# CMU-SAFARI/AirLift

Measured on AMD Instinct MI355X. Metric: reads/sec remapped (150 bp PE), higher is better.
Workload: dtype u8/int32 (int8 SW lanes, u64 hashes)

## Files before the change

airlift_amd/csrc/al_kernels_chain.hip:

```cpp
#include <hip/hip_runtime.h>
#include <stdint.h>
#include "al_internal.h"
#include "al_device.h"

#define CT_TILE 1024
#define CT_SEGS (CT_TILE / 2)
#define CT_FRAGS 32
#define CT_NU_CAP 64
#define CT_CLIN_N 512
#define CT_NONE 0xffffu

#define R_XLO(r) ((uint32_t)(r) & 0xffffu)
#define R_Q(r) ((int32_t)((uint32_t)(r) >> 16 & 0xfffu))
#define R_SEG(r) ((int32_t)((uint32_t)(r) >> 28 & 1u))
#define R_F(r) ((int32_t)(int16_t)((r) >> 32))
#define R_P(r) ((uint32_t)((r) >> 48))
#define ROW_B30 (1u << 30)
#define ROW_B31 (1u << 31)

struct CtFrag {
	uint64_t aoff;
	uint32_t f, na;
	int32_t mdx, mdy; uint32_t drlim;
	uint32_t start;
// ... 684 lines not shown
	const uint32_t f = fb_list[v]; const uint32_t n_u = v_nu[v];
	const uint64_t *su = v_u + v_a_off[v] + v; uint64_t *du = u_all + a_off[f] + f; uint32_t *duo = uo_all + a_off[f] + f;
	uint32_t run = 0;
	for (uint32_t c0 = 0; c0 < n_u; c0 += 64) {
		const uint32_t c = c0 + lane; const uint64_t uc = c < n_u ? su[c] : 0ULL; const uint32_t cnt = (uint32_t)uc;
		uint32_t incl = cnt; for (int d = 1; d < 64; d <<= 1) { const uint32_t t = __shfl_up(incl, d); if (lane >= d) incl += t; }
		if (c < n_u) { du[c] = uc; duo[c] = run + incl - cnt; }
		run += __shfl(incl, 63);
	}
	const AlAnchor *sc = v_chained + v_a_off[v]; AlAnchor *dc = chained + a_off[f];
	for (uint32_t t = lane; t < run; t += 64) dc[t] = sc[t];
	if (lane == 0) frag_nu[f] = n_u;
}

__global__ void __launch_bounds__(256)
k_frag_meta(const uint32_t *__restrict__ frag_first, const uint32_t *__restrict__ rd_len, int n_frag, uint32_t *__restrict__ meta)
{
	const int f = blockIdx.x * blockDim.x + threadIdx.x;
	if (f >= n_frag) return;
	const uint32_t r0 = frag_first[f], r1 = frag_first[f + 1];
	uint32_t q = 0; for (uint32_t r = r0; r < r1; ++r) q += rd_len[r];
	meta[f] = q | (r1 - r0 > 1 ? 1u << 31 : 0u);
}
```

airlift_amd/csrc/al_runtime.h:

```cpp
#pragma once
#include <hip/hip_runtime.h>
#include <stdio.h>
#include <vector>
#include <string>
#include <thread>
#include <chrono>
#include "al_internal.h"
#include "al_stream_plan.h"
#include "al_env.h"
#include "al_devmem.h"

template <typename T> struct DevBuf {
	T *p = nullptr; size_t cap = 0;
	int ensure(size_t n, bool keep = false, hipStream_t s = 0, int line = __builtin_LINE(), const char *file = __builtin_FILE())
	{
		if (n <= cap) return 0;
		al_alloc_site() = AlAllocSite{file, line};
		const size_t big_div = (size_t)al_env().grow_div;
		const size_t ncap = n + (n * sizeof(T) >= ((size_t)256 << 20) ? n / big_div : n / 4) + 64;
		T *np = nullptr;
		if (!keep && p) { al_dev_free(p); p = nullptr; cap = 0; }
		if (al_dev_malloc((void **)&np, ncap * sizeof(T)) != hipSuccess) {
			(void)hipGetLastError();
			fprintf(stderr, "[airlift] device allocation of %zu bytes failed\n", ncap * sizeof(T)); al_nomem_flag() = true; return -1;
// ... 61 lines not shown
	std::vector<uint32_t> h_rd_len, h_frag_first, h_frag_hash;
	std::vector<uint64_t> h_rd_off, h_mini_off;
	std::vector<uint32_t> h_rd_seq;
	std::vector<uint8_t> h_flip;

	DevBuf<uint32_t> rd_seq, rd_len, frag_first, frag_hash, mini_cnt, frag_nm, frag_na, frag_nu, rechain_list, rechain_sorted, tmp_u32;
	DevBuf<uint64_t> rd_off, mini_off, a_off, u, ws_u64, tmp_u64, tmp_u64b;
	DevBuf<uint32_t> uo;
	DevBuf<uint64_t> big_k0, big_k1;
	DevBuf<AlAnchor> v_anchors, v_chained; DevBuf<uint64_t> v_u, v_a_off, v_first64; DevBuf<uint32_t> v_na, v_nseg, v_first, v_rd_len, v_order, v_nu, fbk_list;
	DevBuf<uint64_t> d_uslot; DevBuf<uint32_t> d_rel, d_fragid, cmp_list, ctie, frag_meta, chain_cls;
	DevBuf<int32_t> frag_rep, ws_i32;
	DevBuf<AlAnchor> mini, heap_ws, anchors, chained;
	DevBuf<AlMatch> match;
	DevBuf<unsigned long long> counters;
	DevBuf<uint8_t> scan_tmp;
	DevBuf<uint8_t> big_tmp;
	DevBuf<uint32_t> chain_key, chain_idx, chain_idx2, tie_list, lb_buf;
	DevBuf<AlAnchor> chain_tmp; DevBuf<uint64_t> u_tmp, okey_tmp, seg_first, seg_first0, vs_off, big_off, big_toff;
	DevBuf<uint64_t> vs_res;
	DevBuf<uint32_t> seg_cnt, seg_cnt0, seg_t1, vs_na, vs_meta, vs_cls, seg_key, seg_idx, seg_ord, fb_list, fb2_list, fb3_list, big_na, big_nt, big_tent, big_cuts, tie_frags, tie_sorted, heap_cnt;
	AlChainScratch tie2;
	uint64_t n_chain_fallback = 0;
	uint64_t chain_who[AL_CHAIN_WHO_N] = {};
	DevBuf<unsigned long long> seed_cnt;
	uint64_t seed_who[AL_SEED_WHO_N] = {};
	bool seed_tap_pass1 = false;
	int max_qlen_sum = 0;
	int max_rd_len = 0;
	bool attr_chain_order = false, attr_regs_heavy = false;
	bool no_taps = false;
	bool dev_batch = false;
	DevBuf<uint64_t> a_off_p1; DevBuf<uint32_t> frag_na_p1; DevBuf<int32_t> frag_rep_p1;
	uint64_t n_anchor_total = 0, n_anchor_pass1 = 0;
	double anchor_grow_hw = 1.3;
	uint32_t n_rechain = 0;

	DevBuf<AlReg> regs0, regs;
	DevBuf<uint32_t> reg_cnt, cigar;
	DevBuf<uint64_t> reg_off, cig_off;
	DevBuf<uint8_t> align_ws;
	DevBuf<AlAnchor> seg_a;
	DevBuf<uint64_t> seg_u;
	uint64_t n_regs_cap_total = 0, n_cigar_cap_total = 0;
	bool ran = false;
	uint64_t stat_bytes_in = 0;
	uint32_t stat_n_slow = 0;
	unsigned long long stat_dp_jobs[10] = {}, stat_dp_tbases[10] = {};
	al_batch_stat_t stat;
};

int al_upload_index(const al_idx_t *mi, int device, AlDevIndex *out);
int al_windows_prepare(al_ctx_t *c, int n_tok, int read_len);
// ... 69 lines not shown
```

airlift_amd/csrc/al_runtime.hip:

```cpp
#include <hip/hip_runtime.h>
#include <stdio.h>
#include <stdlib.h>
#include <string.h>
#include <cstring>
#include <algorithm>
#include <functional>
#include <thread>
#include <chrono>
#include "al_internal.h"
#include "al_device.h"
#include <mutex>
#include <vector>
#include "al_runtime.h"
#include "al_prim.h"
#include "al_dev_sort.h"
#include "al_io.h"

extern "C" __global__ void k_sketch(const uint32_t *, const uint64_t *, const uint32_t *, const uint64_t *, AlAnchor *, uint32_t *, int, int, int, int);
extern "C" __global__ void k_seed(const uint64_t *, int, const uint32_t *, const uint32_t *, const uint64_t *, AlAnchor *, const uint32_t *, AlMatch *, uint32_t *, uint32_t *, int32_t *, const uint32_t *, int, int, int, uint32_t *);
#ifndef AL_SPEC_CAP
#define AL_SPEC_CAP 512
#endif
struct SpecOut { AlMatch *match; uint32_t *meta; uint32_t *cnt; uint64_t *cand; uint32_t cap, per, cand_cap; };
struct SpecView { uint32_t *first, *rdlen, *nm, *na, *tie, *list, *n_list; uint64_t *moff, *aoff; };
extern "C" __global__ void k_spec_count(const uint64_t *, int, const uint32_t *, const uint32_t *, const uint64_t *, const AlAnchor *, const uint32_t *, const int32_t *, int, int, uint32_t, SpecOut, int, const uint32_t *);
extern "C" __global__ void k_spec_pick(const uint64_t *, int, const uint32_t *, const uint32_t *, const uint64_t *, const AlAnchor *, const uint32_t *, int, SpecOut);
__global__ void k_spec_layout(const uint32_t *, uint32_t, uint32_t, SpecView);
__global__ void k_spec_mark(const uint32_t *, uint32_t, const uint32_t *, const uint32_t *, uint32_t *, uint32_t *, uint32_t *);
__global__ void k_spec_apply(const uint32_t *, const uint32_t *, const uint64_t *, const AlAnchor *, const uint64_t *, AlAnchor *);
extern "C" __global__ void k_alser_count(const AlAnchor *, const uint64_t *, const uint32_t *, const uint32_t *, const uint32_t *, int, int, unsigned long long *);
extern "C" __global__ void k_rechain_test(const AlAnchor *, const uint64_t *, const uint64_t *, const uint32_t *, const uint32_t *, const int32_t *, const uint32_t *, int, uint32_t *, uint32_t *);
struct TileSched { uint32_t n_items; uint32_t ent[7]; uint32_t item[7]; };
struct CtDefer { uint64_t *off, *uslot; uint32_t *na, *meta, *rel, *fragid, *cls; uint32_t *cnt; uint32_t cap; uint32_t *cmp_list, *cmp_cnt; uint32_t *ctie; };
__global__ void k_frag_meta(const uint32_t *, const uint32_t *, int, uint32_t *);
__global__ void k_chain_tile6(const AlAnchor *, const uint64_t *, const uint32_t *, const uint32_t *, const uint32_t *, const TileSched, const uint32_t *, AlAnchor *, uint64_t *, uint32_t *, uint32_t *, uint32_t *, uint32_t *, const AlParams, const int, unsigned long long *, const int, const CtDefer);
template <int CAP> __global__ void k_chain_coop(const AlAnchor *, AlAnchor *, uint64_t *, uint32_t *, const uint64_t *, const uint32_t *, const uint32_t *, const uint64_t *, const uint32_t *, const uint32_t *, uint32_t *, const uint32_t *, int, const AlParams, unsigned long long *);
__global__ void k_u_compact(const uint32_t *, const uint32_t *, const uint64_t *, uint32_t *, uint64_t *, uint32_t *, const uint32_t *, uint32_t *, uint32_t *);
__global__ void k_uo_fill(const uint32_t *, int, const uint64_t *, const uint32_t *, const uint64_t *, uint32_t *, const uint32_t *);
__global__ void k_fb_meta(const uint32_t *, int, const uint32_t *, const uint32_t *, uint32_t *, uint32_t *);
__global__ void k_fb_reads(const uint32_t *, int, const uint32_t *, const uint32_t *, const uint64_t *, uint32_t *, uint32_t *, uint32_t *);
__global__ void k_fb_copy_in(const uint32_t *, int, const uint64_t *, const uint32_t *, const AlAnchor *, const uint64_t *, AlAnchor *);
__global__ void k_fb_copy_out(const uint32_t *, int, const uint64_t *, const uint64_t *, const uint32_t *, const uint64_t *, const AlAnchor *, uint32_t *, uint64_t *, uint32_t *, AlAnchor *);
template <int CAP> __global__ void k_anchor_sort(const uint64_t *, const uint32_t *, const uint32_t *, const uint64_t *, const AlMatch *, const uint32_t *, const uint32_t *, const uint64_t *, AlAnchor *, uint32_t *, unsigned int *, const uint32_t *, int, unsigned long long *, int);
__global__ void k_anchor_sort_small(const uint64_t *, const uint32_t *, const uint32_t *, const uint64_t *, const AlMatch *, const uint32_t *, const uint32_t *, const uint64_t *, AlAnchor *, uint32_t *, unsigned int *, const uint32_t *, int, unsigned long long *, int);
template <int HCAP, int LANES> __global__ void k_anchor_heap(const uint64_t *, const uint32_t *, const uint32_t *, const uint64_t *, const AlMatch *, const uint32_t *, const uint32_t *, const uint64_t *, AlAnchor *, AlAnchor *, const uint32_t *, const uint32_t *, int, int, unsigned long long *, int, const uint32_t *, uint32_t);
template <int MCAPH, int RING> __global__ void k_anchor_heap_wave(const uint64_t *, const uint32_t *, const uint32_t *, const uint64_t *, const AlMatch *, const uint32_t *, const uint32_t *, const uint64_t *, AlAnchor *, const uint32_t *, const uint32_t *, const uint32_t *, uint32_t, unsigned long long *, int);
template <int NSET, int RING> __global__ void k_anchor_heap_lanes(const uint64_t *, const uint32_t *, const uint32_t *, const uint64_t *, const AlMatch *, const uint32_t *, const uint32_t *, const uint64_t *, AlAnchor *, const uint32_t *, const uint32_t *, const uint32_t *, int, unsigned long long *, int);
template <int CAP> __global__ void k_chain(const AlAnchor *, const uint64_t *, const uint32_t *, const uint32_t *, const uint32_t *, AlAnchor *, uint64_t *, uint32_t *, int32_t *, uint64_t *, const uint32_t *, int, AlParams, unsigned long long *, ChainSeg);
template <int CAPL, int LANES> __global__ void k_chain_lds(const AlAnchor *, const uint64_t *, const uint32_t *, const uint32_t *, const uint32_t *, AlAnchor *, uint64_t *, uint32_t *, uint64_t *, const uint32_t *, int, int, AlParams, unsigned long long *, ChainSeg, uint32_t *, int);
template <int PER, int NW, int MCAP> __global__ void k_anchor_sort_reg(const uint64_t *, const uint32_t *, const uint32_t *, const uint64_t *, const AlMatch *, const uint32_t *, const uint32_t *, const uint64_t *, AlAnchor *, uint32_t *, const uint32_t *, int, int, int);
__global__ void k_anchor_big_expand(const uint64_t *, const uint64_t *, const uint32_t *, const AlMatch *, const uint32_t *, const uint32_t *, int, const uint64_t *, uint64_t *, int, int);
struct RunMergeOut { const uint64_t *a_off, *mini_off; const uint32_t *frag_first, *rd_len; const AlMatch *match; AlAnchor *anchors; uint32_t *tie_list; int rid_bits, mini_span; };
__global__ void k_big_tiles(const uint32_t *, int, uint32_t *, unsigned int *, uint32_t);
template <int PER, int NW, int MCAP> __global__ void k_anchor_run_sort(const uint64_t *, const uint32_t *, const uint64_t *, const AlMatch *, const uint32_t *, const uint32_t *, const uint32_t *, int, const uint64_t *, const uint32_t *, const uint64_t *, uint64_t *, uint32_t *, int, uint32_t, uint32_t);
__global__ void k_big_tile_ent(const uint64_t *, int, uint32_t, uint32_t *);
__global__ void k_anchor_run_cuts(const uint64_t *, const uint32_t *, const uint32_t *, uint32_t, const uint64_t *, const uint64_t *, const uint32_t *, const uint32_t *, int, uint32_t, uint32_t, uint32_t *);
__global__ void k_anchor_run_merge(const uint64_t *, uint64_t *, const uint32_t *, const uint32_t *, const uint32_t *, const uint64_t *, const uint64_t *, const uint32_t *, const uint32_t *, int, RunMergeOut, uint32_t, uint32_t);
// ... 81 lines not shown
	int prio_lo = 0, prio_hi = 0; (void)hipDeviceGetStreamPriorityRange(&prio_lo, &prio_hi);
	const bool side_hi = al_env().side_prio;
	if (hipStreamCreateWithFlags(&c->phys[0], hipStreamNonBlocking) != hipSuccess) { delete c; return nullptr; }
	c->stream = c->phys[0];
	for (int p = 1; p < c->n_phys; ++p) {
		bool side_like = false; for (int r = AL_ROLE_SIDE; r <= AL_ROLE_AUX2; ++r) side_like |= c->role_map[r] == p;
		if (hipStreamCreateWithPriority(&c->phys[p], hipStreamNonBlocking, side_like && side_hi ? prio_hi : 0) != hipSuccess) { delete c; return nullptr; }
	}
	for (int i = 0; i < 4; ++i) if (hipEventCreate(&c->ev_side[i]) != hipSuccess) { delete c; return nullptr; }
	for (int i = 0; i < 2; ++i) if (hipEventCreateWithFlags(&c->ev_fj[i], hipEventDisableTiming) != hipSuccess) { delete c; return nullptr; }
	for (int i = 0; i < 3; ++i) if (hipEventCreateWithFlags(&c->ev_aux[i], hipEventDisableTiming) != hipSuccess) { delete c; return nullptr; }
	for (int i = 0; i < 3; ++i) if (hipEventCreateWithFlags(&c->ev_spec[i], hipEventDisableTiming) != hipSuccess) { delete c; return nullptr; }
	for (int i = 0; i < 5; ++i) if (hipEventCreateWithFlags(&c->ev_ovl[i], hipEventDisableTiming) != hipSuccess) { delete c; return nullptr; }
	if (al_upload_index(mi, device, &c->di) != 0) { delete c; return nullptr; }
	AlParams &P = c->P;
	P.k = mi->k; P.w = mi->w; P.seed = opt->seed; P.bw = opt->bw; P.max_gap = opt->max_gap; P.max_gap_ref = opt->max_gap_ref; P.max_frag_len = opt->max_frag_len;
	P.max_chain_skip = opt->max_chain_skip; P.max_chain_iter = opt->max_chain_iter; P.min_cnt = opt->min_cnt; P.min_chain_score = opt->min_chain_score;
	P.mask_level = opt->mask_level; P.pri_ratio = opt->pri_ratio; P.max_clip_ratio = opt->max_clip_ratio; P.best_n = opt->best_n;
	P.a = opt->a; P.b = opt->b; P.q = opt->q; P.e = opt->e; P.q2 = opt->q2; P.e2 = opt->e2; P.sc_ambi = opt->sc_ambi; P.zdrop = opt->zdrop; P.zdrop_inv = opt->zdrop_inv;
	P.end_bonus = opt->end_bonus; P.min_dp_max = opt->min_dp_max; P.pe_ori = opt->pe_ori; P.pe_bonus = opt->pe_bonus; P.mid_occ = opt->mid_occ; P.max_occ = opt->max_occ;
	const AlEnvCtx ce = al_env_ctx();
	P.dbg = ce.dbg; P.dbg2 = ce.dbg2; P.dp_exit = ce.dp_exit; P.dp_exit_stride = ce.dp_exit_stride;
	if (P.dbg) fprintf(stderr, "[airlift] AL_DBG=%d: timing experiment, results are NOT valid\n", P.dbg);
	if (P.dbg2 & ~32) fprintf(stderr, "[airlift] AL_DBG2=%d: timing experiment, results are NOT valid\n", P.dbg2);
	if (ce.dp_exit_stride_refused) fprintf(stderr, "[airlift] AL_DP_EXIT_STRIDE=%s is not 1, 2, 4 or 8: using 8\n", ce.dp_exit_stride_refused);
	memset(&c->stat, 0, sizeof(c->stat));
	return c;
}

void al_align_state_free(al_ctx_t *c);
static void ctx_release_buffers(al_ctx_t *c)
{
	for (int p = 0; p < c->n_phys; ++p) if (c->phys[p]) (void)hipStreamSynchronize(c->phys[p]);
	(void)hipGetLastError();
	al_align_state_free(c);
	for (int p = 1; p < c->n_phys; ++p) if (c->phys[p]) (void)hipStreamSynchronize(c->phys[p]);
	c->spec_busy = false; c->spec_pending = false; c->n_spec = 0;
	c->spec_match.release(); c->spec_meta.release(); c->spec_cnt.release(); c->spec_use.release(); c->spec_v32.release(); c->spec_v64.release(); c->spec_anchors.release(); c->spec_na2.release(); c->seed_cnt.release();
	if (c->stream) (void)hipStreamSynchronize(c->stream);
	c->rd_seq.release(); c->rd_len.release(); c->frag_first.release(); c->frag_hash.release(); c->mini_cnt.release(); c->frag_nm.release(); c->frag_na.release();
	c->frag_nu.release(); c->rechain_list.release(); c->rechain_sorted.release(); c->tmp_u32.release(); c->rd_off.release(); c->mini_off.release(); c->a_off.release(); c->u.release();
	c->ws_u64.release(); c->tmp_u64.release(); c->frag_rep.release(); c->ws_i32.release(); c->mini.release(); c->heap_ws.release(); c->anchors.release();
	c->chained.release(); c->match.release(); c->counters.release(); c->scan_tmp.release(); c->regs0.release(); c->regs.release(); c->reg_cnt.release();
	c->big_tmp.release(); c->chain_key.release(); c->chain_idx.release(); c->chain_idx2.release(); c->tie_list.release(); c->lb_buf.release(); c->tmp_u64b.release();
	c->chain_tmp.release(); c->u_tmp.release(); c->okey_tmp.release(); c->fb2_list.release(); c->fb3_list.release(); c->seg_cnt.release(); c->seg_first.release(); c->seg_cnt0.release(); c->seg_first0.release(); c->seg_t1.release(); c->vs_off.release(); c->vs_na.release(); c->vs_meta.release(); c->vs_res.release(); c->vs_cls.release(); c->seg_key.release(); c->seg_idx.release(); c->seg_ord.release(); c->fb_list.release(); c->tie_frags.release(); c->heap_cnt.release(); c->tie_sorted.release(); c->big_na.release(); c->big_off.release();
	c->uo.release(); c->big_k0.release(); c->big_k1.release(); c->v_anchors.release(); c->v_chained.release(); c->v_u.release(); c->v_a_off.release(); c->v_first64.release(); c->v_na.release(); c->v_nseg.release(); c->v_first.release(); c->v_rd_len.release(); c->v_order.release(); c->v_nu.release(); c->fbk_list.release(); c->d_uslot.release(); c->d_rel.release(); c->chain_cls.release(); c->d_fragid.release(); c->cmp_list.release(); c->ctie.release(); c->frag_meta.release(); c->tie2.release();
	c->big_nt.release(); c->big_toff.release(); c->big_tent.release(); c->big_cuts.release();
// ... 205 lines not shown
};
template <class S> static ChainRound chain_round(S &from, hipStream_t s, bool own, bool company, uint32_t *fb_cnt, uint32_t *cnts, uint64_t n_anchor, int n_frag_max)
{
	return ChainRound{s, own, company, nullptr, fb_cnt, cnts, n_anchor, n_frag_max,
#define X(n) from.n,
		CHAIN_SCRATCH(X)
#undef X
	};
}
static ChainRound round_main(al_ctx_t *c, bool company = false) { return chain_round(*c, c->stream, false, company, (uint32_t *)(c->counters.p + 15), (uint32_t *)(c->counters.p + 16), c->n_anchor_total, c->n_frag); }
static ChainRound round_beside(al_ctx_t *c, uint64_t n_anchor, int n_frag_max) { AlChainScratch &T = c->tie2; return chain_round(T, c->on(AL_ROLE_SIDE), true, true, T.cnt.p, T.cnt.p + 4, n_anchor, n_frag_max); }

static int lower_bounds(al_ctx_t *c, const uint32_t *keys, uint32_t n, const uint32_t *thr, int nt, uint32_t *out, const ChainRound *R = nullptr)
{
	hipStream_t const s = R ? R->s : c->stream; DevBuf<uint32_t> &lb_buf = R ? R->lb_buf : c->lb_buf;
	if (lb_buf.ensure(16)) return -1;
	uint32_t init[16]; LbThr T; T.n = nt;
	for (int i = 0; i < 16; ++i) { init[i] = n; T.v[i] = i < nt ? thr[i] : 0xffffffffu; }
	AL_HIP_CHECK(hipMemcpyAsync(lb_buf.p, init, 64, hipMemcpyHostToDevice, s));
	if (n > 0) hipLaunchKernelGGL(k_lower_bounds, dim3((n + 255) / 256), dim3(256), 0, s, keys, n, T, lb_buf.p);
	if (R) return R->fetch(out, lb_buf.p, 4 * (size_t)nt);
	AL_HIP_CHECK(hipMemcpyAsync(out, lb_buf.p, 4 * nt, hipMemcpyDeviceToHost, s));
	AL_HIP_CHECK(hipStreamSynchronize(s));
	return 0;
}

static int chain_by_segments(al_ctx_t *c, const ChainRound &R, const AlBatchPtrs &B, const uint32_t *order, int n, bool lds_ok, bool first, const uint32_t *skip_flag, bool with_keys = false, int big_from = 0 , int big8_from = 0 )
{
	hipStream_t s = R.s;
	auto ev = [&](int st) -> int { if (first) AL_HIP_CHECK(hipEventRecord(c->ev[st + 1], s)); return 0; };
	if (n <= 0) { if (ev(ST_SEG_FIND) || ev(ST_SEG_CHAIN_LDS) || ev(ST_SEG_CHAIN_WAVE) || ev(ST_SEG_MERGE)) return -1; return 0; }
	int lmin = c->opt.min_cnt > 1 ? c->opt.min_cnt : 1;
	{ const int per = c->mi->k + 1, need = (c->opt.min_chain_score + per - 1) / per; if (need > lmin) lmin = need; }
	if (R.need(R.seg_cnt, (size_t)n + 2) || R.need(R.seg_first, (size_t)n + 2) || R.need(R.seg_cnt0, (size_t)n + 2) || R.need(R.seg_first0, (size_t)n + 2)) return -1;
	const std::optional<int> &seg_big = al_env().test_seg_big;
	const int segs_big = seg_big.value_or(8192), segm_big = seg_big ? std::max(1, *seg_big / 8) : 1024;
	if (seg_big) { big_from = 0; big8_from = 0; c->chain_who[CW_SEG_BIG] += (uint64_t)n; }
	if (big8_from < 0 || big8_from > n) big8_from = 0;
	if (n > big8_from) hipLaunchKernelGGL(HIP_KERNEL_NAME(k_seg_scan<8>), dim3(n - big8_from), dim3(512), 0, s, B.anchors, B.a_off, B.frag_na, B.frag_first, B.rd_len, order + big8_from, n - big8_from, c->P, lmin, 0,
	                   (const uint64_t *)nullptr, (const uint64_t *)nullptr, R.seg_cnt.p + big8_from, R.seg_cnt0.p + big8_from, (uint64_t *)nullptr, (uint32_t *)nullptr, (uint32_t *)nullptr, skip_flag,
	                   (uint32_t *)nullptr, (uint32_t *)nullptr, (uint32_t *)nullptr, big8_from, segs_big);
	hipLaunchKernelGGL(HIP_KERNEL_NAME(k_seg_scan<1>), dim3(n), dim3(64), 0, s, B.anchors, B.a_off, B.frag_na, B.frag_first, B.rd_len, order, n, c->P, lmin, 0,
	                   (const uint64_t *)nullptr, (const uint64_t *)nullptr, R.seg_cnt.p, R.seg_cnt0.p, (uint64_t *)nullptr, (uint32_t *)nullptr, (uint32_t *)nullptr, skip_flag,
	                   (uint32_t *)nullptr, (uint32_t *)nullptr, (uint32_t *)nullptr, big8_from, segs_big);
	AL_HIP_CHECK(hipMemsetAsync(R.seg_cnt.p + n, 0, 4, s)); AL_HIP_CHECK(hipMemsetAsync(R.seg_cnt0.p + n, 0, 4, s));
	if (R.scan(R.seg_cnt.p, R.seg_first.p, n) || R.scan(R.seg_cnt0.p, R.seg_first0.p, n)) return -1;
// ... 138 lines not shown
	if (S.n_items > 0) {
		const int force_fb = al_env().test_tile_fb ? 1 : 0;
		if (cap >= (1ULL << 31)) { fprintf(stderr, "[airlift] too many anchors in one batch for the deferred-segment list: upload fewer fragments\n"); al_nomem_flag() = true; return -1; }
		if (R.need(R.vs_off, cap) || R.need(R.d_uslot, cap) || R.need(R.vs_na, cap) || R.need(R.vs_meta, cap) || R.need(R.d_rel, cap) || R.need(R.d_fragid, cap) || R.need(R.vs_cls, cap) ||
		    R.need(R.cmp_list, (size_t)R.n_frag_max + 2) || R.need(R.ctie, (size_t)c->n_frag + 2)) return -1;
		AL_HIP_CHECK(hipMemsetAsync(cnts, 0, 16, s));
		AL_HIP_CHECK(hipMemsetAsync(R.ctie.p, 0, ((size_t)c->n_frag + 1) * 4, s));
		CtDefer D; D.off = R.vs_off.p; D.uslot = R.d_uslot.p; D.na = R.vs_na.p; D.meta = R.vs_meta.p; D.rel = R.d_rel.p; D.fragid = R.d_fragid.p; D.cls = R.vs_cls.p; D.cnt = cnts + 1; D.cap = (uint32_t)cap;
		D.cmp_list = R.cmp_list.p; D.cmp_cnt = cnts + 2; D.ctie = R.ctie.p;
		hipLaunchKernelGGL(k_chain_tile6, dim3(S.n_items), dim3(256), 0, s, c->anchors.p, c->a_off.p, c->frag_na.p, c->frag_meta.p, list, S, skip_flag,
		                   c->chained.p, c->u.p, c->uo.p, c->frag_nu.p, R.fb_list.p, cnts, c->P, lmin, c->counters.p, force_fb, D);
		if (ev(ST_SEG_FIND)) return -1;
		if (c->ovl_pending && !R.own) { AL_HIP_CHECK(hipStreamWaitEvent(s, c->ev_ovl[3], 0)); c->ovl_pending = false; }
	} else if (ev(ST_SEG_FIND)) return -1;
	if (beside) AL_HIP_CHECK(hipEventRecord(c->ev_fj[1], s));
	auto finish = [&]() -> int {
	if (S.n_items > 0) {
		if (al_env().trace) { const hipError_t e = hipStreamSynchronize(s); fprintf(stderr, "[airlift] trace: tile kernel (%u items, first pass %d) -> %s\n", S.n_items, (int)first, hipGetErrorName(e)); }
		uint32_t h[3] = {0, 0, 0};
		if (R.fetch(h, cnts, 12)) return -1;
		const uint32_t n_def = h[1], n_cmp = h[2]; n_def_t = n_def; n_cmp_t = n_cmp;
		c->chain_who[CW_TILE_ITEMS] += S.n_items; c->chain_who[CW_TILE_FRAGS] += S.ent[6] - S.ent[0]; c->chain_who[CW_DEFERRED] += n_def; c->chain_who[CW_COMPACTED] += n_cmp;
		if (n_def > cap) { fprintf(stderr, "[airlift] deferred-segment list overflow (%u > %zu)\n", n_def, cap); return -1; }
		if (n_def > 0) {
			if (R.need(R.seg_key, (size_t)n_def + 1) || R.need(R.seg_ord, (size_t)n_def + 1) || R.need(R.seg_t1, (size_t)n_def + 1)) return -1;
			hipLaunchKernelGGL(k_iota_u32, dim3((n_def + 255) / 256), dim3(256), 0, s, R.seg_t1.p, n_def);
			if (R.prim([&](void *t, size_t &b) { return rocprim::radix_sort_pairs(t, b, (const uint32_t *)R.vs_cls.p, R.seg_key.p, (const uint32_t *)R.seg_t1.p, R.seg_ord.p, (int)n_def, 0, 4, s); })) return -1;
			static const uint32_t thr[8] = {1, 2, 3, 4, 5, 6, 7, 8};
			uint32_t lb[8];
			if (lower_bounds(c, R.seg_key.p, n_def, thr, 8, lb, &R)) return -1;
			const uint32_t cb[10] = {0, lb[0], lb[1], lb[2], lb[3], lb[4], lb[5], lb[6], lb[7], n_def};
			static const uint32_t capl0[9] = {16, 24, 32, 40, 48, 64, 80, 96, 128};
			for (int k = 0; k < 9; ++k) n_cls_t += cb[k + 1] > cb[k];
			const int coop_env = al_env().chain_coop;
			bool thin[9]; thin[0] = false;
			for (int k = 1; k < 9; ++k) thin[k] = coop_env == 1 || (coop_env != 0 && cb[k + 1] - cb[k] < 4096u);
			uint32_t capl[9]; for (int k = 0; k < 9; ++k) capl[k] = thin[k] ? 0u : capl0[k];
			size_t wsb[10]; wsb[0] = 0; for (int k = 0; k < 9; ++k) wsb[k + 1] = wsb[k] + (size_t)(cb[k + 1] - cb[k]) * capl[k];
			if (R.need(R.ws_u64, wsb[9] + 64)) return -1;
			if (al_env().trace && first) fprintf(stderr, "[airlift] trace: tile chaining: %u items, %u deferred segments (<=16:%u <=24:%u <=32:%u <=40:%u <=48:%u <=64:%u <=80:%u <=96:%u <=128:%u), %u fragments to compact\n", S.n_items, n_def,
			                          cb[1] - cb[0], cb[2] - cb[1], cb[3] - cb[2], cb[4] - cb[3], cb[5] - cb[4], cb[6] - cb[5], cb[7] - cb[6], cb[8] - cb[7], cb[9] - cb[8], n_cmp);
			ChainSeg sg{R.vs_meta.p, nullptr, nullptr, 0, nullptr, R.d_uslot.p, R.d_rel.p, R.d_fragid.p, R.ctie.p};
#define LDEF(C, L, K) do { if (!thin[K]) LCH(C, L, -1, R.vs_off.p, R.vs_na.p, c->chained.p, c->u.p, (uint32_t *)nullptr, R.seg_ord.p + cb[K], (int)(cb[K + 1] - cb[K]), sg, c->uo.p, R.ws_u64.p + wsb[K], C); } while (0)
			const bool two = al_env().chain_ovl2 && c->n_frag < 400000 && !R.own;
			hipStream_t const s_cls[2] = {s, two ? c->on(AL_ROLE_OVL2) : s};
			if (two) { AL_HIP_CHECK(hipEventRecord(c->ev_ovl[4], s)); AL_HIP_CHECK(hipStreamWaitEvent(c->on(AL_ROLE_OVL2), c->ev_ovl[4], 0)); }
			{ int turn = 0;
#define LDEF2(C, L, K) do { if (!thin[K] && cb[K + 1] > cb[K]) { hipStream_t const s = s_cls[turn++ & 1]; LDEF(C, L, K); } } while (0)
			LDEF2(16, 64, 0); LDEF2(24, 64, 1); LDEF2(32, 64, 2); LDEF2(40, 64, 3); LDEF2(48, 64, 4); LDEF2(64, 64, 5); LDEF2(80, 64, 6); LDEF2(96, 64, 7); LDEF2(128, 32, 8);
#undef LDEF2
			}
			if (two) { AL_HIP_CHECK(hipEventRecord(c->ev_ovl[4], c->on(AL_ROLE_OVL2))); AL_HIP_CHECK(hipStreamWaitEvent(s, c->ev_ovl[4], 0)); }
			for (int k = 1; k < 9; ) {
				if (!thin[k]) { ++k; continue; }
				int k1 = k; while (k1 + 1 < 9 && thin[k1 + 1]) ++k1;
				const int nn = (int)(cb[k1 + 1] - cb[k]);
				if (nn > 0) {
					c->chain_who[CW_DEFERRED_COOP] += (uint64_t)nn;
					if (k1 <= 4) hipLaunchKernelGGL(HIP_KERNEL_NAME(k_chain_coop<48>), dim3((nn + 3) / 4), dim3(64), 0, s, c->anchors.p, c->chained.p, c->u.p, c->uo.p, R.vs_off.p, R.vs_na.p, R.vs_meta.p, R.d_uslot.p, R.d_rel.p, R.d_fragid.p, R.ctie.p,
					                                (const uint32_t *)R.seg_ord.p + cb[k], nn, c->P, c->counters.p);
					else hipLaunchKernelGGL(HIP_KERNEL_NAME(k_chain_coop<128>), dim3((nn + 3) / 4), dim3(64), 0, s, c->anchors.p, c->chained.p, c->u.p, c->uo.p, R.vs_off.p, R.vs_na.p, R.vs_meta.p, R.d_uslot.p, R.d_rel.p, R.d_fragid.p, R.ctie.p,
					                        (const uint32_t *)R.seg_ord.p + cb[k], nn, c->P, c->counters.p);
				}
// ... 569 lines not shown
extern "C" int al_dbg_chain(al_ctx_t *c, const uint64_t *anchors_xy, const uint64_t *a_off, const uint32_t *tie_flag, uint32_t *nu_out, uint64_t *u_out, uint32_t *uo_out, uint64_t *chained_xy, uint64_t *counts)
{
	if (!c || c->dev_batch || c->n_frag <= 0 || (int)c->h_frag_first.size() < c->n_frag + 1 || !c->frag_first.p) { fprintf(stderr, "[airlift] al_dbg_chain: needs a batch uploaded with al_batch_upload\n"); return -1; }
	const int nf = c->n_frag;
	if (a_off[0] != 0) return -2;
	for (int f = 0; f < nf; ++f) if (a_off[f + 1] < a_off[f] || a_off[f + 1] - a_off[f] > 0x7fffffffu) return -2;
	const uint64_t total = a_off[nf];
	AL_HIP_CHECK(hipSetDevice(c->device));
	al_nomem_flag() = false;
	hipStream_t s = c->stream;
	std::vector<uint32_t> na((size_t)nf + 1, 0u);
	for (int f = 0; f < nf; ++f) na[f] = (uint32_t)(a_off[f + 1] - a_off[f]);
	c->n_anchor_pass1 = total; c->n_anchor_total = total; c->n_rechain = 0; c->ran = false; c->n_chain_fallback = 0;
	if (ensure_anchor_space(c, total + 1, false) || c->frag_meta.ensure((size_t)nf + 1) || c->chain_key.ensure(nf + 1) || c->chain_idx.ensure(nf + 1) || c->chain_idx2.ensure(nf + 1) || c->tie_list.ensure((size_t)nf + 2)) return -1;
	AL_HIP_CHECK(hipMemsetAsync(c->counters.p, 0, 32 * sizeof(unsigned long long), s));
	if (total) AL_HIP_CHECK(hipMemcpyAsync(c->anchors.p, anchors_xy, (size_t)total * 16, hipMemcpyHostToDevice, s));
	AL_HIP_CHECK(hipMemcpyAsync(c->a_off.p, a_off, ((size_t)nf + 1) * 8, hipMemcpyHostToDevice, s));
	AL_HIP_CHECK(hipMemcpyAsync(c->frag_na.p, na.data(), ((size_t)nf + 1) * 4, hipMemcpyHostToDevice, s));
	AL_HIP_CHECK(hipMemsetAsync(c->tie_list.p, 0, ((size_t)nf + 1) * 4, s));
	AL_HIP_CHECK(hipMemcpyAsync(c->tie_list.p, tie_flag, (size_t)nf * 4, hipMemcpyHostToDevice, s));
	AL_HIP_CHECK(hipStreamSynchronize(s));
	hipLaunchKernelGGL(k_frag_meta, dim3((nf + 255) / 256), dim3(256), 0, s, c->frag_first.p, c->rd_len.p, nf, c->frag_meta.p);
	for (int i = 0; i < CW_N; ++i) c->chain_who[i] = 0;
	ChainPlan pl;
	if (chain_plan(c, nullptr, nf, true, pl)) return -1;
	AL_HIP_CHECK(hipEventRecord(c->ev_ovl[2], s));
	if (chain_small(c, pl) || chain_rounds(c, pl, nullptr)) return -1;
	for (int p = 0; p < c->n_phys; ++p) if (c->phys[p]) AL_HIP_CHECK(hipStreamSynchronize(c->phys[p]));
	AL_HIP_CHECK(hipStreamSynchronize(s));
	AL_HIP_CHECK(hipGetLastError());
	AL_HIP_CHECK(hipMemcpy(nu_out, c->frag_nu.p, (size_t)nf * 4, hipMemcpyDeviceToHost));
	AL_HIP_CHECK(hipMemcpy(u_out, c->u.p, (size_t)(total + nf + 1) * 8, hipMemcpyDeviceToHost));
	AL_HIP_CHECK(hipMemcpy(uo_out, c->uo.p, (size_t)(total + nf + 1) * 4, hipMemcpyDeviceToHost));
	if (total) AL_HIP_CHECK(hipMemcpy(chained_xy, c->chained.p, (size_t)total * 16, hipMemcpyDeviceToHost));
	if (al_env().test_guard && al_dev_guard_check()) fprintf(stderr, "[airlift] GUARD: violations after al_dbg_chain\n");
	if (counts) {
		for (int i = 0; i < CW_N; ++i) counts[i] = c->chain_who[i];
		counts[CW_N] = c->n_chain_fallback; counts[CW_N + 1] = pl.lds_ok; counts[CW_N + 2] = pl.tiles_ok; counts[CW_N + 3] = pl.tile_from;
		counts[CW_N + 4] = pl.lb1; counts[CW_N + 5] = pl.lb65; counts[CW_N + 6] = pl.lb129; counts[CW_N + 7] = (uint64_t)pl.lmin;
	}
	return 0;
}

extern "C" int al_dbg_seed(al_ctx_t *c, const uint32_t *list, int n_list, uint64_t *counts)
{
	if (!c || c->dev_batch || c->n_frag <= 0 || (int)c->h_frag_first.size() < c->n_frag + 1 || !c->frag_first.p) { fprintf(stderr, "[airlift] al_dbg_seed: needs a batch uploaded with al_batch_upload\n"); return -1; }
// ... 116 lines not shown
	return 0;
}

extern "C" int64_t al_dbg_copy(al_ctx_t *c, const char *name, void *dst, int64_t max_bytes)
{
	if (!c) return -1;
	const void *src = nullptr; int64_t bytes = 0; const bool p1 = c->n_rechain > 0;
	const int64_t nf = c->n_frag, nr = c->n_reads;
	if (!strcmp(name, "mini")) src = c->mini.p, bytes = (int64_t)c->mini_total * 16;
	else if (!strcmp(name, "mini_cnt")) src = c->mini_cnt.p, bytes = nr * 4;
	else if (!strcmp(name, "frag_na")) src = c->frag_na.p, bytes = nf * 4;
	else if (!strcmp(name, "frag_na_p1")) src = p1 ? c->frag_na_p1.p : c->frag_na.p, bytes = nf * 4;
	else if (!strcmp(name, "frag_nm")) src = c->frag_nm.p, bytes = nf * 4;
	else if (!strcmp(name, "tie_list")) src = c->tie_list.p, bytes = c->tie_list.p ? nf * 4 : 0;
	else if (!strcmp(name, "frag_rep")) src = c->frag_rep.p, bytes = nf * 4;
	else if (!strcmp(name, "frag_rep_p1")) src = p1 ? c->frag_rep_p1.p : c->frag_rep.p, bytes = nf * 4;
	else if (!strcmp(name, "frag_nu")) src = c->frag_nu.p, bytes = nf * 4;
	else if (!strcmp(name, "a_off")) src = c->a_off.p, bytes = (nf + 1) * 8;
	else if (!strcmp(name, "a_off_p1")) src = p1 ? c->a_off_p1.p : c->a_off.p, bytes = (nf + 1) * 8;
	else if (!strcmp(name, "anchors")) src = c->anchors.p, bytes = (int64_t)c->n_anchor_total * 16;
	else if (!strcmp(name, "chained")) src = c->chained.p, bytes = (int64_t)c->n_anchor_total * 16;
	else if (!strcmp(name, "u")) src = c->u.p, bytes = (int64_t)(c->n_anchor_total + nf + 1) * 8;
	else if (!strcmp(name, "uo")) src = c->uo.p, bytes = (int64_t)(c->n_anchor_total + nf + 1) * 4;
	else if (!strcmp(name, "mini_off") && !c->dev_batch) { bytes = (nr + 1) * 8; if (bytes > max_bytes) bytes = max_bytes; memcpy(dst, c->h_mini_off.data(), bytes); return bytes; }
	else if (!strcmp(name, "mini_off")) src = c->mini_off.p, bytes = (nr + 1) * 8;
	else return -1;
	if (bytes > max_bytes) bytes = max_bytes;
	if (hipSetDevice(c->device) != hipSuccess) return -1;
	if (bytes > 0 && hipMemcpy(dst, src, bytes, hipMemcpyDeviceToHost) != hipSuccess) return -1;
	return bytes;
}

extern "C" int al_batch_upload_flat(al_ctx_t *c, int n_frag, const int *n_segs, const int *qlens, const char *seq_concat, const char *name_prefix, int64_t first_index)
{
	int nr = 0; for (int f = 0; f < n_frag; ++f) nr += n_segs[f];
	std::vector<const char *> seqs(nr), names(nr); std::vector<std::string> nm(n_frag);
	const char *p = seq_concat; int r = 0;
	for (int f = 0; f < n_frag; ++f) {
		nm[f] = std::string(name_prefix ? name_prefix : "") + std::to_string(first_index + f);
		for (int j = 0; j < n_segs[f]; ++j, ++r) { seqs[r] = p; p += qlens[r]; names[r] = nm[f].c_str(); }
	}
	return al_batch_upload(c, n_frag, n_segs, qlens, seqs.data(), names.data());
}

#include "al_bam.h"
int al_sort_keys(al_ctx_t *c, const uint64_t *keys, uint32_t *perm, size_t n)
// ... 109 lines not shown
```

Before: 16.21 million.

## Sort deferred chain segments by length within windows to cut lane divergence

Adds a device kernel that stably counting-sorts the deferred-segment order by anchor count inside fixed windows, and by default (code 7) applies it with a 16384-entry window starting after the first class. Grouping segments of similar length means each wavefront in the per-class chaining kernels wastes fewer lanes waiting on the longest segment, since work scales roughly with n². It costs one extra kernel launch with large LDS use (a raised dynamic shared-memory limit) and it changes the processing order of segments. It also adds trace diagnostics and taps for the deferred order.

```diff
diff --git a/airlift_amd/csrc/al_dev_defer_order.h b/airlift_amd/csrc/al_dev_defer_order.h
--- /dev/null
+++ b/airlift_amd/csrc/al_dev_defer_order.h
@@ -0,0 +1,31 @@
+#pragma once
+#include <stddef.h>
+#include <stdint.h>
+#include <algorithm>
+
+static constexpr int al_defer_order_bits = 0x700;
+static constexpr int al_defer_order_default = 7;
+static constexpr uint32_t al_window_whole = 0xffffffffu, al_window_max = 16384u;
+static inline int al_defer_order_code(int dbg2) { const int c = (dbg2 >> 8) & 7; return c == 0 ? al_defer_order_default : c; }
+static inline uint32_t al_defer_order_window(int dbg2)
+{
+	switch (al_defer_order_code(dbg2)) {
+	case 2: return 64u;
+	case 3: return 1024u;
+	case 4: return 4096u;
+	case 5: case 7: return al_window_max;
+	case 6: return al_window_whole;
+	default: return 0u;
+	}
+}
+static inline int al_defer_order_first_class(int dbg2) { return al_defer_order_code(dbg2) == 7 ? 1 : 0; }
+
+static inline void al_window_order_host(uint32_t *list, const uint32_t *len_of, size_t n, size_t W)
+{
+	if (W == 0) return;
+	for (size_t b = 0; b < n; b += W) {
+		const size_t e = n - b < W ? n : b + W;
+		std::stable_sort(list + b, list + e, [len_of](uint32_t x, uint32_t y) { return len_of[x] < len_of[y]; });
+		if (e == n) break;
+	}
+}
diff --git a/airlift_amd/csrc/al_kernels_chain.hip b/airlift_amd/csrc/al_kernels_chain.hip
--- a/airlift_amd/csrc/al_kernels_chain.hip
+++ b/airlift_amd/csrc/al_kernels_chain.hip
@@ -730,3 +730,52 @@
 	uint32_t q = 0; for (uint32_t r = r0; r < r1; ++r) q += rd_len[r];
 	meta[f] = q | (r1 - r0 > 1 ? 1u << 31 : 0u);
 }
+
+#define WO_NW 4
+static_assert(WO_NW * 64 == 256, "k_window_order: thread t scans the counts of key t (8-bit keys)");
+__global__ void __launch_bounds__(64 * WO_NW)
+k_window_order(uint32_t *__restrict__ list, const uint32_t *__restrict__ len_of, uint32_t n, uint32_t W)
+{
+	extern __shared__ uint32_t wo_lds[];
+	__shared__ uint32_t s_wsum[WO_NW];
+	uint32_t *const s_idx = wo_lds, *const s_cnt = wo_lds + W; uint8_t *const s_key = reinterpret_cast<uint8_t *>(s_cnt + WO_NW * 256);
+	const uint32_t base = blockIdx.x * W;
+	if (base >= n) return;
+	const uint32_t cnt = n - base < W ? n - base : W;
+	const uint32_t per = (cnt + 64u * WO_NW - 1u) / (64u * WO_NW) * 64u;
+	const uint32_t t = threadIdx.x, lane = t & 63u, w = t >> 6;
+	for (uint32_t i = t; i < WO_NW * 256u; i += 64u * WO_NW) s_cnt[i] = 0u;
+	__syncthreads();
+	for (uint32_t i = t; i < cnt; i += 64u * WO_NW) {
+		const uint32_t e = list[base + i], l = len_of[e], k = l < 255u ? l : 255u;
+		s_idx[i] = e; s_key[i] = (uint8_t)k; atomicAdd(&s_cnt[(i / per) * 256u + k], 1u);
+	}
+	__syncthreads();
+	{
+		uint32_t c[WO_NW], tot = 0u;
+#pragma unroll
+		for (int j = 0; j < WO_NW; ++j) { c[j] = s_cnt[j * 256 + t]; tot += c[j]; }
+		uint32_t incl = tot;
+		for (int d = 1; d < 64; d <<= 1) { const uint32_t v = __shfl_up(incl, d); if (lane >= (uint32_t)d) incl += v; }
+		if (lane == 63u) s_wsum[w] = incl;
+		__syncthreads();
+		uint32_t off = incl - tot; for (uint32_t j = 0; j < w; ++j) off += s_wsum[j];
+#pragma unroll
+		for (int j = 0; j < WO_NW; ++j) { s_cnt[j * 256 + t] = off; off += c[j]; }
+	}
+	__syncthreads();
+	uint32_t *const my_cnt = s_cnt + w * 256u;
+	for (uint32_t i0 = 0; i0 < per; i0 += 64u) {
+		const uint32_t i = w * per + i0 + lane; const bool on = i < cnt;
+		const uint32_t k = on ? s_key[i] : 0u;
+		unsigned long long m = __ballot(on);
+#pragma unroll
+		for (int b = 0; b < 8; ++b) { const bool bit = (k >> b) & 1u; const unsigned long long bal = __ballot(bit); m &= bit ? bal : ~bal; }
+		const uint32_t rank = (uint32_t)__popcll(m & ((1ULL << lane) - 1ULL));
+		const uint32_t pos = on ? my_cnt[k] + rank : 0u;
+		__syncthreads();
+		if (on && rank == 0u) my_cnt[k] += (uint32_t)__popcll(m);
+		__syncthreads();
+		if (on) list[base + pos] = s_idx[i];
+	}
+}
diff --git a/airlift_amd/csrc/al_runtime.h b/airlift_amd/csrc/al_runtime.h
--- a/airlift_amd/csrc/al_runtime.h
+++ b/airlift_amd/csrc/al_runtime.h
@@ -107,13 +107,14 @@
 	DevBuf<uint32_t> seg_cnt, seg_cnt0, seg_t1, vs_na, vs_meta, vs_cls, seg_key, seg_idx, seg_ord, fb_list, fb2_list, fb3_list, big_na, big_nt, big_tent, big_cuts, tie_frags, tie_sorted, heap_cnt;
 	AlChainScratch tie2;
 	uint64_t n_chain_fallback = 0;
+	uint32_t tap_def_n = 0;
 	uint64_t chain_who[AL_CHAIN_WHO_N] = {};
 	DevBuf<unsigned long long> seed_cnt;
 	uint64_t seed_who[AL_SEED_WHO_N] = {};
 	bool seed_tap_pass1 = false;
 	int max_qlen_sum = 0;
 	int max_rd_len = 0;
-	bool attr_chain_order = false, attr_regs_heavy = false;
+	bool attr_chain_order = false, attr_regs_heavy = false, attr_window_order = false;
 	bool no_taps = false;
 	bool dev_batch = false;
 	DevBuf<uint64_t> a_off_p1; DevBuf<uint32_t> frag_na_p1; DevBuf<int32_t> frag_rep_p1;
diff --git a/airlift_amd/csrc/al_runtime.hip b/airlift_amd/csrc/al_runtime.hip
--- a/airlift_amd/csrc/al_runtime.hip
+++ b/airlift_amd/csrc/al_runtime.hip
@@ -11,10 +11,12 @@
 #include "al_device.h"
 #include <mutex>
 #include <vector>
+#include <string>
 #include "al_runtime.h"
 #include "al_prim.h"
 #include "al_dev_sort.h"
 #include "al_io.h"
+#include "al_dev_defer_order.h"
 
 extern "C" __global__ void k_sketch(const uint32_t *, const uint64_t *, const uint32_t *, const uint64_t *, AlAnchor *, uint32_t *, int, int, int, int);
 extern "C" __global__ void k_seed(const uint64_t *, int, const uint32_t *, const uint32_t *, const uint64_t *, AlAnchor *, const uint32_t *, AlMatch *, uint32_t *, uint32_t *, int32_t *, const uint32_t *, int, int, int, uint32_t *);
@@ -33,6 +35,7 @@
 struct TileSched { uint32_t n_items; uint32_t ent[7]; uint32_t item[7]; };
 struct CtDefer { uint64_t *off, *uslot; uint32_t *na, *meta, *rel, *fragid, *cls; uint32_t *cnt; uint32_t cap; uint32_t *cmp_list, *cmp_cnt; uint32_t *ctie; };
 __global__ void k_frag_meta(const uint32_t *, const uint32_t *, int, uint32_t *);
+__global__ void k_window_order(uint32_t *, const uint32_t *, uint32_t, uint32_t);
 __global__ void k_chain_tile6(const AlAnchor *, const uint64_t *, const uint32_t *, const uint32_t *, const uint32_t *, const TileSched, const uint32_t *, AlAnchor *, uint64_t *, uint32_t *, uint32_t *, uint32_t *, uint32_t *, const AlParams, const int, unsigned long long *, const int, const CtDefer);
 template <int CAP> __global__ void k_chain_coop(const AlAnchor *, AlAnchor *, uint64_t *, uint32_t *, const uint64_t *, const uint32_t *, const uint32_t *, const uint64_t *, const uint32_t *, const uint32_t *, uint32_t *, const uint32_t *, int, const AlParams, unsigned long long *);
 __global__ void k_u_compact(const uint32_t *, const uint32_t *, const uint64_t *, uint32_t *, uint64_t *, uint32_t *, const uint32_t *, uint32_t *, uint32_t *);
@@ -160,7 +163,7 @@
 	const AlEnvCtx ce = al_env_ctx();
 	P.dbg = ce.dbg; P.dbg2 = ce.dbg2; P.dp_exit = ce.dp_exit; P.dp_exit_stride = ce.dp_exit_stride;
 	if (P.dbg) fprintf(stderr, "[airlift] AL_DBG=%d: timing experiment, results are NOT valid\n", P.dbg);
-	if (P.dbg2 & ~32) fprintf(stderr, "[airlift] AL_DBG2=%d: timing experiment, results are NOT valid\n", P.dbg2);
+	if (P.dbg2 & ~(32 | al_defer_order_bits)) fprintf(stderr, "[airlift] AL_DBG2=%d: timing experiment, results are NOT valid\n", P.dbg2);
 	if (ce.dp_exit_stride_refused) fprintf(stderr, "[airlift] AL_DP_EXIT_STRIDE=%s is not 1, 2, 4 or 8: using 8\n", ce.dp_exit_stride_refused);
 	memset(&c->stat, 0, sizeof(c->stat));
 	return c;
@@ -412,6 +415,52 @@
 	if (R) return R->fetch(out, lb_buf.p, 4 * (size_t)nt);
 	AL_HIP_CHECK(hipMemcpyAsync(out, lb_buf.p, 4 * nt, hipMemcpyDeviceToHost, s));
 	AL_HIP_CHECK(hipStreamSynchronize(s));
+	return 0;
+}
+
+static int window_order(al_ctx_t *c, hipStream_t s, uint32_t *list, const uint32_t *len_of, uint32_t n, uint32_t W)
+{
+	if (W == 0 || W == al_window_whole || n < 2) return 0;
+	if (W > n) W = (n + 63u) & ~63u;
+	if (W > al_window_max || (W & 63u)) { fprintf(stderr, "[airlift] internal: window of %u entries\n", W); return -1; }
+	const size_t lds = (size_t)W * 5 + 4 * 256 * 4;
+	if (lds > 65536 && !c->attr_window_order) { AL_HIP_CHECK(hipFuncSetAttribute((const void *)k_window_order, hipFuncAttributeMaxDynamicSharedMemorySize, (int)((size_t)al_window_max * 5 + 4096))); c->attr_window_order = true; }
+	hipLaunchKernelGGL(k_window_order, dim3((n + W - 1) / W), dim3(256), lds, s, list, len_of, n, W);
+	return 0;
+}
+
+static int trace_defer_order(const ChainRound &R, bool first, const uint32_t *ord, const uint32_t *na, uint32_t n_def, const uint32_t *cb, uint32_t W_on)
+{
+	std::vector<uint32_t> h_ord(n_def), h_na(n_def), L;
+	AL_HIP_CHECK(hipStreamSynchronize(R.s));
+	AL_HIP_CHECK(hipMemcpy(h_ord.data(), ord, (size_t)n_def * 4, hipMemcpyDeviceToHost));
+	AL_HIP_CHECK(hipMemcpy(h_na.data(), na, (size_t)n_def * 4, hipMemcpyDeviceToHost));
+	uint32_t hist[129] = {};
+	for (uint32_t i = 0; i < n_def; ++i) ++hist[std::min(h_na[i], 128u)];
+	std::string hs;
+	for (int l = 9; l <= 128; ++l) { char b[24]; snprintf(b, sizeof b, " %u", hist[l]); hs += b; }
+	fprintf(stderr, "[airlift] trace: round %s (first pass %d): deferred segments by length 9 ... 128:%s\n", R.tag(), (int)first, hs.c_str());
+	static const uint32_t Ws[5] = {0, 1024, 4096, al_window_max, al_window_whole};
+	double paid0 = 0;
+	for (int wi = 0; wi < 5; ++wi) {
+		L = h_ord;
+		al_window_order_host(L.data(), h_na.data(), L.size(), Ws[wi] == al_window_whole ? L.size() : Ws[wi]);
+		double used_t = 0, paid_t = 0; char b[64]; std::string ls;
+		for (int k = 0; k < 9; ++k) {
+			const uint32_t lanes = k == 8 ? 32u : 64u; double used = 0, paid = 0;
+			for (uint32_t i = cb[k]; i < cb[k + 1]; i += lanes) {
+				uint32_t nmax = 0;
+				for (uint32_t j = i; j < std::min(i + lanes, cb[k + 1]); ++j) { const uint32_t n = h_na[L[j]]; used += (double)n * (n - 1); nmax = std::max(nmax, n); }
+				paid += (double)lanes * nmax * (nmax - 1);
+			}
+			snprintf(b, sizeof b, " %.3f", paid > 0 ? used / paid : 0.0); ls += b;
+			used_t += used; paid_t += paid;
+		}
+		if (wi == 0) paid0 = paid_t;
+		snprintf(b, sizeof b, "%u", Ws[wi]);
+		fprintf(stderr, "[airlift] trace: round %s (first pass %d): lane utilisation, window %s%s: classes%s, total %.3f, pairs paid for %.4g (%.3f of the class order's)\n", R.tag(), (int)first,
+		        Ws[wi] == al_window_whole ? "whole list" : Ws[wi] ? b : "off", Ws[wi] == W_on ? " *" : "", ls.c_str(), paid_t > 0 ? used_t / paid_t : 0.0, paid_t, paid0 > 0 ? paid_t / paid0 : 0.0);
+	}
 	return 0;
 }
 
@@ -596,14 +645,19 @@
 		const uint32_t n_def = h[1], n_cmp = h[2]; n_def_t = n_def; n_cmp_t = n_cmp;
 		c->chain_who[CW_TILE_ITEMS] += S.n_items; c->chain_who[CW_TILE_FRAGS] += S.ent[6] - S.ent[0]; c->chain_who[CW_DEFERRED] += n_def; c->chain_who[CW_COMPACTED] += n_cmp;
 		if (n_def > cap) { fprintf(stderr, "[airlift] deferred-segment list overflow (%u > %zu)\n", n_def, cap); return -1; }
+		if (!R.own && skip_flag) c->tap_def_n = n_def;
 		if (n_def > 0) {
+			const uint32_t W = al_defer_order_window(c->P.dbg2); const bool whole = W == al_window_whole;
 			if (R.need(R.seg_key, (size_t)n_def + 1) || R.need(R.seg_ord, (size_t)n_def + 1) || R.need(R.seg_t1, (size_t)n_def + 1)) return -1;
 			hipLaunchKernelGGL(k_iota_u32, dim3((n_def + 255) / 256), dim3(256), 0, s, R.seg_t1.p, n_def);
-			if (R.prim([&](void *t, size_t &b) { return rocprim::radix_sort_pairs(t, b, (const uint32_t *)R.vs_cls.p, R.seg_key.p, (const uint32_t *)R.seg_t1.p, R.seg_ord.p, (int)n_def, 0, 4, s); })) return -1;
-			static const uint32_t thr[8] = {1, 2, 3, 4, 5, 6, 7, 8};
+			if (R.prim([&](void *t, size_t &b) { return rocprim::radix_sort_pairs(t, b, whole ? (const uint32_t *)R.vs_na.p : (const uint32_t *)R.vs_cls.p, R.seg_key.p, (const uint32_t *)R.seg_t1.p, R.seg_ord.p, (int)n_def, 0, whole ? 8 : 4, s); })) return -1;
+			static const uint32_t thr_cls[8] = {1, 2, 3, 4, 5, 6, 7, 8}, thr_len[8] = {17, 25, 33, 41, 49, 65, 81, 97};
 			uint32_t lb[8];
-			if (lower_bounds(c, R.seg_key.p, n_def, thr, 8, lb, &R)) return -1;
+			if (lower_bounds(c, R.seg_key.p, n_def, whole ? thr_len : thr_cls, 8, lb, &R)) return -1;
 			const uint32_t cb[10] = {0, lb[0], lb[1], lb[2], lb[3], lb[4], lb[5], lb[6], lb[7], n_def};
+			if (al_env().trace && trace_defer_order(R, first, R.seg_ord.p, R.vs_na.p, n_def, cb, W)) return -1;
+			const uint32_t w_from = cb[al_defer_order_first_class(c->P.dbg2)];
+			if (window_order(c, s, R.seg_ord.p + w_from, R.vs_na.p, n_def - w_from, W)) return -1;
 			static const uint32_t capl0[9] = {16, 24, 32, 40, 48, 64, 80, 96, 128};
 			for (int k = 0; k < 9; ++k) n_cls_t += cb[k + 1] > cb[k];
 			const int coop_env = al_env().chain_coop;
@@ -612,7 +666,7 @@
 			uint32_t capl[9]; for (int k = 0; k < 9; ++k) capl[k] = thin[k] ? 0u : capl0[k];
 			size_t wsb[10]; wsb[0] = 0; for (int k = 0; k < 9; ++k) wsb[k + 1] = wsb[k] + (size_t)(cb[k + 1] - cb[k]) * capl[k];
 			if (R.need(R.ws_u64, wsb[9] + 64)) return -1;
-			if (al_env().trace && first) fprintf(stderr, "[airlift] trace: tile chaining: %u items, %u deferred segments (<=16:%u <=24:%u <=32:%u <=40:%u <=48:%u <=64:%u <=80:%u <=96:%u <=128:%u), %u fragments to compact\n", S.n_items, n_def,
+			if (al_env().trace) fprintf(stderr, "[airlift] trace: tile chaining, round %s (first pass %d): %u items, %u deferred segments (<=16:%u <=24:%u <=32:%u <=40:%u <=48:%u <=64:%u <=80:%u <=96:%u <=128:%u), %u fragments to compact\n", R.tag(), (int)first, S.n_items, n_def,
 			                          cb[1] - cb[0], cb[2] - cb[1], cb[3] - cb[2], cb[4] - cb[3], cb[5] - cb[4], cb[6] - cb[5], cb[7] - cb[6], cb[8] - cb[7], cb[9] - cb[8], n_cmp);
 			ChainSeg sg{R.vs_meta.p, nullptr, nullptr, 0, nullptr, R.d_uslot.p, R.d_rel.p, R.d_fragid.p, R.ctie.p};
 #define LDEF(C, L, K) do { if (!thin[K]) LCH(C, L, -1, R.vs_off.p, R.vs_na.p, c->chained.p, c->u.p, (uint32_t *)nullptr, R.seg_ord.p + cb[K], (int)(cb[K + 1] - cb[K]), sg, c->uo.p, R.ws_u64.p + wsb[K], C); } while (0)
@@ -1228,6 +1282,7 @@
 	AL_HIP_CHECK(hipStreamSynchronize(s));
 	hipLaunchKernelGGL(k_frag_meta, dim3((nf + 255) / 256), dim3(256), 0, s, c->frag_first.p, c->rd_len.p, nf, c->frag_meta.p);
 	for (int i = 0; i < CW_N; ++i) c->chain_who[i] = 0;
+	c->tap_def_n = 0;
 	ChainPlan pl;
 	if (chain_plan(c, nullptr, nf, true, pl)) return -1;
 	AL_HIP_CHECK(hipEventRecord(c->ev_ovl[2], s));
@@ -1390,6 +1445,9 @@
 	else if (!strcmp(name, "chained")) src = c->chained.p, bytes = (int64_t)c->n_anchor_total * 16;
 	else if (!strcmp(name, "u")) src = c->u.p, bytes = (int64_t)(c->n_anchor_total + nf + 1) * 8;
 	else if (!strcmp(name, "uo")) src = c->uo.p, bytes = (int64_t)(c->n_anchor_total + nf + 1) * 4;
+	else if (!strcmp(name, "def_n")) { bytes = 4; if (bytes > max_bytes) bytes = max_bytes; memcpy(dst, &c->tap_def_n, bytes); return bytes; }
+	else if (!strcmp(name, "def_ord")) src = c->seg_ord.p, bytes = (int64_t)c->tap_def_n * 4;
+	else if (!strcmp(name, "def_na")) src = c->vs_na.p, bytes = (int64_t)c->tap_def_n * 4;
 	else if (!strcmp(name, "mini_off") && !c->dev_batch) { bytes = (nr + 1) * 8; if (bytes > max_bytes) bytes = max_bytes; memcpy(dst, c->h_mini_off.data(), bytes); return bytes; }
 	else if (!strcmp(name, "mini_off")) src = c->mini_off.p, bytes = (nr + 1) * 8;
 	else return -1;
```

New measurement: 16.32 million (median of 6 runs). About the same (+0.7%).
